# RIVM-bioinformatics/auriclass

Measured on AMD Instinct MI355X. Metric: Gbases/s sketched (k=21, s=1000), higher is better.
Workload: dtype u64; 1 GPU; synthetic FASTQ 10000000 x 150 bp reads per GPU from a 12000000 bp genome, 0.5% substitutions, 3150000000 bytes resident in HBM; k=21, s=1000, min_multiplicity=1, total_bases=1500000000, ranks=1, parallelism=1 GPU

## Files before the change

auriclass_amd/csrc/mhx_sketch.hip:

```cpp
#include "mhx_block.h"
#include "mhx_device.h"
#include "mhx_screen.h"
#include "mhx_tile.h"

#include <type_traits>

namespace mhx {

struct DeviceInserter {
    unsigned long long *keys;
    uint32_t *cnts;
    uint64_t mask;
    unsigned long long *stats;
    __device__ __forceinline__ void operator()(uint64_t h)
    {
        if (h == kEmptyKey) {
            atomicAdd(&stats[kStatMaxKey], 1ull);
            return;
        }
        uint64_t slot = h & mask;
        for (int probe = 0; probe < 8192; ++probe) {
            const unsigned long long prev = atomicCAS(&keys[slot], (unsigned long long)kEmptyKey, (unsigned long long)h);
            if (prev == kEmptyKey || prev == h) {
                atomicAdd(&cnts[slot], 1u);
                return;
            }
            slot = (slot + 1) & mask;
        }
        atomicOr(&stats[kStatFlags], (unsigned long long)kFlagTableFull);
    }
};

struct ScreenProber {
    unsigned long long *keys;
    uint32_t *cnts;
    uint64_t mask;
    unsigned long long *stats;
    __device__ __forceinline__ void operator()(uint64_t h)
    {
        if (h == kEmptyKey) {
            atomicAdd(&stats[kStatMaxKey], 1ull);
            return;
        }
        const uint64_t at = screen_find(reinterpret_cast<const uint64_t *>(keys), mask, h);
        if (at != kScreenAbsent && !screen_count_stands(atomicAdd(&cnts[at], 1u))) {
            atomicSub(&cnts[at], 1u);
            atomicOr(&stats[kStatFlags], (unsigned long long)kFlagCountWrap);
        }
    }
};

template <int K, class Ins> __device__ __noinline__ uint32_t finish_candidate(const TileSmem &sm, uint32_t code, uint64_t T, Ins ins)
{
    return process_deferred<K>(sm, code, T, ins);
}

struct CandidateQueue {
    TileSmem &sm;
    uint32_t first, cap;
    __device__ __forceinline__ void operator()(uint32_t group, int window) const
    {
        const uint32_t slot = atomicAdd(&sm.misc[7], 1u);
        if (slot < cap) sm.list[first + slot] = (uint16_t)((group << 3) | (uint32_t)window);
    }
};

__device__ __forceinline__ uint64_t ld_state(const uint64_t *p)
{
    return __hip_atomic_load(p, __ATOMIC_RELAXED, __HIP_MEMORY_SCOPE_AGENT);
}
__device__ __forceinline__ void st_state(uint64_t *p, uint64_t v)
{
    __hip_atomic_store(p, v, __ATOMIC_RELAXED, __HIP_MEMORY_SCOPE_AGENT);
}

__device__ uint32_t lookback_wave(uint64_t *state, uint32_t tile, uint32_t first_tile, uint32_t agg,
                                  unsigned long long *stats)
{
    const int lane = threadIdx.x & 63;
    constexpr uint64_t A = 1ull << 32, P = 2ull << 32;
    if (tile == first_tile) {
        if (lane == 0) st_state(&state[tile], P | agg);
        return 0;
    }
    if (lane == 0) st_state(&state[tile], A | agg);
    uint32_t excl = 0;
    int64_t pos = (int64_t)tile - 1;
    constexpr int kWin = 4;
    bool done = false;
    for (uint32_t spins = 0; !done;) {
        uint64_t w[kWin];
#pragma unroll
        for (int j = 0; j < kWin; ++j) {
            const int64_t idx = pos - lane - 64 * j;
            w[j] = idx >= (int64_t)first_tile ? ld_state(&state[idx]) : P;
        }
        bool blocked = false;
#pragma unroll
        for (int j = 0; j < kWin; ++j) {
            if (done || blocked) continue;
            const uint32_t f = (uint32_t)(w[j] >> 32);
            const uint64_t notready = __ballot(f == 0);
            const uint64_t isp = __ballot(f == 2);
            uint64_t take = 0;
            if (isp) {
                const int q = __builtin_ctzll(isp);
                const uint64_t below = q ? (~0ull >> (64 - q)) : 0ull;
                if ((notready & below) == 0) {
                    take = below | (1ull << q);
                    done = true;
                }
            } else if (!notready) {
                take = ~0ull;
            }
            if (take) {
                uint32_t v = ((take >> lane) & 1ull) ? (uint32_t)w[j] : 0u;
#pragma unroll
                for (int o = 32; o > 0; o >>= 1) v += __shfl_xor(v, o);
                excl += v;
                if (!done) pos -= 64;
            } else {
                blocked = true;
            }
        }
        if (blocked) {
            if (++spins > (1u << 20)) {
                if (lane == 0) atomicOr(&stats[kStatFlags], (unsigned long long)kFlagSpinTimeout);
                break;
            }
            __builtin_amdgcn_s_sleep(4);
        }
    }
    if (lane == 0) st_state(&state[tile], P | (uint64_t)(excl + agg));
    return excl;
}

#ifdef MHX_PARSE_LOOPS
constexpr bool kParseLoops = true;
#else
constexpr bool kParseLoops = false;
#endif
#ifndef MHX_MIN_WAVES
#define MHX_MIN_WAVES 7
#endif
template <int K, int FMT, bool QUEUE, bool PROBE, bool SPLIT = false> __global__ __launch_bounds__(kBlock, MHX_MIN_WAVES) void sketch_tile_kernel(const HashArgs a)
{
    __shared__ TileSmem sm;
    constexpr bool FASTQ = (FMT != 0), LOOKBACK = (FMT == 1), SELFSYNC = (FMT == 2);
    const int tid = threadIdx.x;
    __builtin_amdgcn_s_setprio(3);

    static_assert(!SPLIT || (!LOOKBACK && !QUEUE && !PROBE), "split launches: inline sketch kernels of formats 0 and 2");
    const uint32_t split_log2 = SPLIT ? (uint32_t)__builtin_ctz(a.split) : 0u;
    const uint32_t slice = SPLIT ? blockIdx.x & (a.split - 1u) : 0u;
    const uint32_t it0 = slice * kBlock + (uint32_t)tid, it_step = (uint32_t)kBlock << split_log2;
    const bool once = slice == 0;
    uint32_t tile;
    if (LOOKBACK) {
        if (tid == 0) sm.misc[2] = a.tile0 + atomicAdd(a.ticket, 1u);
        __syncthreads();
        tile = sm.misc[2];
    } else {
        tile = a.tile0 + (blockIdx.x >> split_log2);
    }
    const uint64_t tile_off = (uint64_t)tile * kTileBytes;
    unsigned long long *stats = reinterpret_cast<unsigned long long *>(a.stats) + (tile % kStatReplicas) * kStatCount;
    if (tid == 0) { sm.misc[3] = 0; sm.misc[4] = 0; sm.misc[5] = 0; sm.misc[7] = 0; }
#ifdef MHX_STAMPS
    uint64_t stamp_prev = clock64();
    int stamp_idx = 0;
#define MHX_STAMP()                                                                                      \
    do {                                                                                                 \
        if (tid == 0) {                                                                                  \
            const uint64_t now_ = clock64();                                                             \
            atomicAdd(&stats[kStatStamp0 + stamp_idx], (unsigned long long)(now_ - stamp_prev));         \
            stamp_prev = now_;                                                                           \
        }                                                                                                \
        ++stamp_idx;                                                                                     \
    } while (0)
#else
#define MHX_STAMP() do { } while (0)
#endif

    phase_stage(sm, tid, a.base, tile_off, a.end);
    __syncthreads();
    MHX_STAMP();

    ThreadState st;
    const bool interior = tile_off >= a.begin && tile_off + kTileBytes + kHaloBytes <= a.end;
    phase_classify(sm, tid, st, tile_off, a.begin, a.end, interior);

    MHX_STAMP();
    uint32_t line_base = 0, excl = 0, tile_total = 0;
    bool fast_parse = false;
    const uint64_t span_left = a.end > tile_off ? a.end - tile_off : 0;
    const uint32_t check_limit = span_left < (uint64_t)(kTileBytes + kHaloBytes) ? (uint32_t)span_left : (uint32_t)(kTileBytes + kHaloBytes);
    if (FASTQ) {
        excl = block_scan_excl<kBlock>(st.nlcount, sm.cnt, tile_total);
        fast_parse = !kParseLoops && parse_events_fit(tile_total);
        if (fast_parse) phase_events(sm, tid, st, excl);
        if (tid == 0) sm.misc[0] = tile == a.first_tile ? 0u : phase_selfsync(sm, check_limit);
        __syncthreads();
        const uint32_t self_phase = sm.misc[0];
        if (SELFSYNC) {
            if (self_phase == 4u) {
                if (tid == 0 && once) { a.phase_rec[tile - a.first_tile] = 0; atomicOr(a.need_lookback, 1u); }
                return;
            }
            if (tid == 0 && once) a.phase_rec[tile - a.first_tile] = phase_record(self_phase, tile_total);
            line_base = self_phase;
        } else {
            if (a.repair && self_phase != 4u) {
                if (tid == 0) {
                    st_state(&a.tile_state[tile], (2ull << 32) | (uint64_t)(self_phase + tile_total));
                    a.phase_rec[tile - a.first_tile] = phase_record(self_phase, tile_total);
                }
                return;
            }
            if (tid < 64) {
                const uint32_t lb = lookback_wave(a.tile_state, tile, a.first_tile, tile_total, stats);
                if (tid == 0) sm.misc[0] = lb;
            }
            __syncthreads();
            line_base = sm.misc[0];
            if (a.repair && tid == 0) a.phase_rec[tile - a.first_tile] = phase_record(line_base, tile_total);
        }
    }
    MHX_STAMP();
    bool bad = false;
    const uint32_t long_records = fast_parse
        ? phase_good_events(sm, tid, st, line_base, excl, tile_total, check_limit, bad, tile_off, a.end, (uint32_t)K)
        : phase_good<FASTQ>(sm, tid, st, line_base, excl, tile_total, check_limit, bad, tile_off, a.end, (uint32_t)K);
    if (FASTQ && bad && once) atomicOr(&stats[kStatFlags], (unsigned long long)kFlagBadFastq);
    if (FASTQ && long_records) atomicAdd(&sm.misc[5], long_records);
    __syncthreads();
    MHX_STAMP();

    uint32_t items = 0;
    const uint32_t kmers = phase_runs<K>(sm, tid, items);
    if (kmers) atomicAdd(&sm.misc[3], kmers);
    uint32_t nitems = 0;
    const uint32_t items_before = block_scan_excl<kBlock>(items, sm.cnt + 8, nitems);
    phase_compact(sm, tid, items_before);
    __syncthreads();
    MHX_STAMP();
    __builtin_amdgcn_s_setprio(0);

    const uint64_t T = *a.thresh;
    const uint32_t limit = admission_limit(T);
    std::conditional_t<PROBE, ScreenProber, DeviceInserter> ins{reinterpret_cast<unsigned long long *>(a.keys), a.cnts, a.slot_mask, stats};
    const uint32_t qcap = (uint32_t)kGroupsPerTile - nitems;
    CandidateQueue queue{sm, nitems, qcap};
    uint32_t ninsert = 0;
    const TailLutPtr lut = hot_tail_table<K>();
    constexpr bool kPairs = pair_words_form<K>(FMT, QUEUE);
    for (uint32_t it = it0; it < nitems; it += it_step) ninsert += process_group<K, QUEUE, kPairs>(sm, sm.list[it], T, limit, ins, queue, lut);
    if (QUEUE) {
        __syncthreads();
        const uint32_t ncand = sm.misc[7];
        if (ncand <= qcap) {
            for (uint32_t c = tid; c < ncand; c += kBlock) ninsert += finish_candidate<K>(sm, sm.list[nitems + c], T, ins);
        } else {
            for (uint32_t it = it0; it < nitems; it += it_step) {
                const uint32_t g = sm.list[it];
                uint32_t vmask = reinterpret_cast<const uint8_t *>(sm.valid)[g];
                while (vmask) {
                    const uint32_t j = (uint32_t)__builtin_ctz(vmask);
                    vmask &= vmask - 1u;
                    ninsert += finish_candidate<K>(sm, (g << 3) | j, T, ins);
                }
            }
        }
    }
    if (ninsert) atomicAdd(&sm.misc[4], ninsert);
    __syncthreads();
    MHX_STAMP();
    if (tid == 0) {
        if (once && sm.misc[3]) atomicAdd(&stats[kStatKmers], (unsigned long long)sm.misc[3]);
        if (sm.misc[4]) atomicAdd(&stats[kStatInserts], (unsigned long long)sm.misc[4]);
        if (once && FASTQ && tile_total) atomicAdd(&stats[kStatLines], (unsigned long long)tile_total);
        if (once && FASTQ && sm.misc[5]) atomicAdd(&stats[kStatRecords], (unsigned long long)sm.misc[5]);
    }
}

template <int K> static hipError_t launch_k(int fmt, const HashArgs &a, hipStream_t st)
{
    if (a.split > 1) {
        if (fmt == 1 || a.queue_candidates || a.probe) return hipErrorInvalidValue;
        if (fmt == 2) hipLaunchKernelGGL((sketch_tile_kernel<K, 2, false, false, true>), dim3(a.ntiles * a.split), dim3(kBlock), 0, st, a);
        else hipLaunchKernelGGL((sketch_tile_kernel<K, 0, false, false, true>), dim3(a.ntiles * a.split), dim3(kBlock), 0, st, a);
        return hipGetLastError();
    }
    const unsigned grid = a.ntiles;
#define MHX_LAUNCH_FORM(FMT_, QUEUE_) do { if (a.probe) hipLaunchKernelGGL((sketch_tile_kernel<K, FMT_, QUEUE_, true>), dim3(grid), dim3(kBlock), 0, st, a); \
                                           else hipLaunchKernelGGL((sketch_tile_kernel<K, FMT_, QUEUE_, false>), dim3(grid), dim3(kBlock), 0, st, a); } while (0)
#define MHX_LAUNCH(FMT_) do { if (a.queue_candidates) MHX_LAUNCH_FORM(FMT_, true); else MHX_LAUNCH_FORM(FMT_, false); } while (0)
    if (fmt == 1) MHX_LAUNCH(1);
    else if (fmt == 2) MHX_LAUNCH(2);
    else MHX_LAUNCH(0);
#undef MHX_LAUNCH
#undef MHX_LAUNCH_FORM
    return hipGetLastError();
}

#ifdef MHX_ONLY_K
#define MHX_K_LIST(X) X(MHX_ONLY_K)
#else
#define MHX_K_LIST(X) X(1) X(2) X(3) X(4) X(5) X(6) X(7) X(8) X(9) X(10) X(11) X(12) X(13) X(14) X(15) X(16) \
    X(17) X(18) X(19) X(20) X(21) X(22) X(23) X(24) X(25) X(26) X(27) X(28) X(29) X(30) X(31) X(32)
#endif

bool hash_k_supported(int k) { return k >= 1 && k <= 32; }

hipError_t launch_hash(int k, int fmt, const HashArgs &a, hipStream_t st)
{
    if (a.ntiles == 0) return hipSuccess;
    if (a.split == 0 || (a.split & (a.split - 1)) || a.split > 8 || (uint64_t)a.ntiles * a.split > 0x7FFFFFFFull) return hipErrorInvalidValue;
    switch (k) {
#define X(KK) case KK: return launch_k<KK>(fmt, a, st);
        MHX_K_LIST(X)
#undef X
    default: return hipErrorInvalidValue;
    }
}

}
```

auriclass_amd/csrc/mhx_tile.h:

```cpp
#pragma once
#include <stdint.h>
#include <type_traits>

#include "mhx_hd.h"
#include "mhx_device_consts.h"
#include "mhx_tail_lut.h"

#define MHX_UNLIKELY(x) __builtin_expect(!!(x), 0)

namespace mhx {

constexpr int kMapWords = (kTileBytes + kHaloBytes) / 32 + 2;
struct TileSmem {
    uint4 bytes[(kTileBytes + kHaloBytes) / 16];
    uint32_t valid[kGroupsPerTile / 4];
    union {
        uint16_t list[kGroupsPerTile];
        uint32_t maps[2 * kMapWords];
    };
    uint32_t cnt[16];
    uint32_t misc[8];
};

MHX_HD uint32_t *tile_nlmap(TileSmem &sm) { return sm.maps; }
// ... 199 lines not shown
{
    const uint32_t lo = (uint32_t)k, hi = (uint32_t)(k >> 32);
    return make64(lo ^ (hi >> 1), hi);
}
MHX_HD uint64_t times5_plus(uint64_t h, uint32_t c)
{
#if defined(__HIP_DEVICE_COMPILE__)
    uint64_t r;
    asm("v_lshl_add_u64 %0, %1, 2, %1" : "=v"(r) : "v"(h));
    return r + c;
#else
    const uint32_t lo = (uint32_t)h, hi = (uint32_t)(h >> 32);
    const uint64_t t = (uint64_t)lo * 5u + c;
    return make64((uint32_t)t, ((hi << 2) + hi) + (uint32_t)(t >> 32));
#endif
}
MHX_HD uint64_t rotated(uint64_t x) { return opaque64(x); }
template <uint64_t C> MHX_HD uint64_t mul64c(uint64_t x, uint32_t &zero)
{
#if defined(__HIP_DEVICE_COMPILE__) && defined(MHX_ASM_MUL64)
    const uint32_t lo = (uint32_t)x, hi = (uint32_t)(x >> 32);
    uint64_t p, carry;
    uint32_t y;
    asm("v_mul_lo_u32 v71, %[lo], %[chi]\n\t"
        "v_mul_lo_u32 %[y], %[hi], %[clo]\n\t"
        "v_add_u32_e32 v71, v71, %[y]\n\t"
        "v_mad_u64_u32 %[p], %[c], %[lo], %[clo], v[70:71]"
        : [p] "=&v"(p), [c] "=&s"(carry), [y] "=&v"(y), "+{v70}"(zero)
        : [lo] "v"(lo), [hi] "v"(hi), [clo] "s"((uint32_t)C), [chi] "s"((uint32_t)(C >> 32))
        : "v71");
    return p;
#else
    (void)zero;
    return opaque64(x * C);
#endif
}
constexpr uint64_t kFmixC2 = 0xc4ceb9fe1a85ec53ull;
MHX_HD uint64_t fmix64_head(uint64_t k, uint32_t &zero)
{
    k = xorshift33(k);
    k = mul64c<0xff51afd7ed558ccdull>(k, zero);
    return xorshift33(k);
}
struct Murmur3Tail {
    uint64_t ka, kb;
    MHX_HD uint64_t finish() const
    {
        uint32_t zero = 0;
        return xorshift33(mul64c<kFmixC2>(ka, zero)) + xorshift33(mul64c<kFmixC2>(kb, zero));
    }
    MHX_HD uint32_t low32() const
    {
        uint32_t zero = 0;
        return (uint32_t)xorshift33(mul64c<kFmixC2>(ka, zero)) + (uint32_t)xorshift33(mul64c<kFmixC2>(kb, zero));
    }
    MHX_HD uint32_t high_bound() const { return (uint32_t)(((ka + kb) * kFmixC2) >> 32) + 1u; }
};
MHX_HD uint32_t admission_limit(uint64_t T)
{
    const uint32_t th = (uint32_t)(T >> 32);
    return th >= 0xFFFFFFFDu ? 0xFFFFFFFFu : th + 2u;
}
template <int K> MHX_HD uint64_t xor_tail_len(uint64_t h, uint64_t k)
{
    h = opaque64(h);
    return make64(xor3((uint32_t)h, (uint32_t)k, (uint32_t)K), (uint32_t)(h >> 32) ^ (uint32_t)(k >> 32));
}
constexpr uint64_t kMurmurSeed = 42;
template <int K> constexpr bool tail_lut_applies() { return K > 16 && (K & 7) >= 1 && (K & 7) <= 5; }
template <int K> constexpr bool hot_tail_lut()
{
#if defined(__HIP_DEVICE_COMPILE__) && !defined(MHX_NO_TAIL_LUT)
    return tail_lut_applies<K>();
#else
    return false;
#endif
}
template <int K> MHX_HD TailLutPtr tail_lut_of() { return tail_lut_table<K & 7, ((K & 15) > 8)>(); }
template <int K, bool LUT> MHX_HD Murmur3Tail murmur3_blocks(const uint32_t (&w)[8], uint64_t k_lut)
{
    static_assert(!LUT || tail_lut_applies<K>(), "no table for this K");
    constexpr uint64_t c1 = kMurmurC1, c2 = kMurmurC2;
    constexpr int NBLK = K / 16, TAIL = K & 15;
    uint64_t h1 = kMurmurSeed, h2 = kMurmurSeed;
    uint32_t zero = 0;
#pragma unroll
    for (int b = 0; b < NBLK; ++b) {
        uint64_t k1 = make64(w[4 * b], w[4 * b + 1]);
        uint64_t k2 = make64(w[4 * b + 2], w[4 * b + 3]);
        k1 = rotl64<31>(mul64c<c1>(k1, zero)); k1 = mul64c<c2>(k1, zero); h1 ^= k1;
        h1 = rotated(rotl64<27>(h1));
        static_assert(0x52dce729ull + 5ull * kMurmurSeed <= 0xFFFFFFFFull, "folded constant of block 0 must fit times5_plus' 32-bit addend");
        if (b == 0) h1 = times5_plus(h1, (uint32_t)(0x52dce729ull + 5ull * kMurmurSeed));
        else { h1 += h2; h1 = times5_plus(h1, 0x52dce729u); }
        k2 = rotl64<33>(mul64c<c2>(k2, zero)); k2 = mul64c<c1>(k2, zero); h2 ^= k2;
        h2 = rotated(rotl64<31>(h2)); h2 += h1; h2 = times5_plus(h2, 0x38495ab5u);
    }
    if (TAIL > 8) {
        uint64_t k2 = make64(w[(4 * NBLK + 2) & 7], w[(4 * NBLK + 3) & 7]);
        if constexpr (LUT) k2 = k_lut;
        else { k2 = rotl64<33>(mul64c<c2>(k2, zero)); k2 = mul64c<c1>(k2, zero); }
        h2 = xor_tail_len<K>(h2, k2);
    } else {
        h2 ^= (uint64_t)K;
    }
    if (TAIL > 0) {
        uint64_t k1 = make64(w[(4 * NBLK) & 7], w[(4 * NBLK + 1) & 7]);
        if constexpr (LUT && TAIL <= 8) k1 = k_lut;
        else { k1 = rotl64<31>(mul64c<c1>(k1, zero)); k1 = mul64c<c2>(k1, zero); }
        h1 = xor_tail_len<K>(h1, k1);
    } else {
        h1 ^= (uint64_t)K;
    }
    h1 += h2; h2 += h1;
    uint64_t ka = fmix64_head(h1, zero), kb = fmix64_head(h2, zero);
    if (K > 16) { ka = opaque64(ka); kb = opaque64(kb); }
    return Murmur3Tail{ka, kb};
}
template <int K, bool LUT = false> MHX_HD Murmur3Tail murmur3_core(const uint32_t (&w)[8], TailLutPtr lut = nullptr)
{
    uint64_t k_lut = 0;
    if constexpr (LUT) k_lut = lut[tail_lut_index<K & 7>(w[(K / 8) * 2], w[((K / 8) * 2 + 1) & 7])];
    return murmur3_blocks<K, LUT>(w, k_lut);
}
template <int K> MHX_HD uint64_t murmur3_h1(const uint32_t (&w)[8]) { return murmur3_core<K>(w).finish(); }


MHX_HD void phase_stage(TileSmem &sm, int tid, const uint8_t *base, uint64_t tile_off, uint64_t end)
{
    const uint64_t lim = (end + 15) & ~(uint64_t)15;
    constexpr int kChunks = kTileBytes / 16;
#ifndef MHX_STAGE_SERIAL
    if (tile_off + (uint64_t)(kTileBytes + kHaloBytes) <= lim) {
        const uint4 *src = reinterpret_cast<const uint4 *>(base + tile_off) + tid;
        uint4 v[kChunks / kBlock], h = {0, 0, 0, 0};
#pragma unroll
        for (int j = 0; j < kChunks / kBlock; ++j) v[j] = src[j * kBlock];
        if (tid < kHaloBytes / 16) h = src[kChunks];
#pragma unroll
        for (int j = 0; j < kChunks / kBlock; ++j) sm.bytes[j * kBlock + tid] = v[j];
        if (tid < kHaloBytes / 16) sm.bytes[kChunks + tid] = h;
        return;
    }
#endif
#pragma unroll
    for (int j = 0; j < kChunks / kBlock; ++j) {
        const int c = j * kBlock + tid;
        const uint64_t off = tile_off + (uint64_t)c * 16;
        uint4 v = {0, 0, 0, 0};
        if (off < lim) v = *reinterpret_cast<const uint4 *>(base + off);
        sm.bytes[c] = v;
    }
    if (tid < kHaloBytes / 16) {
        const int c = kChunks + tid;
        const uint64_t off = tile_off + (uint64_t)c * 16;
        uint4 v = {0, 0, 0, 0};
        if (off < lim) v = *reinterpret_cast<const uint4 *>(base + off);
        sm.bytes[c] = v;
    }
}

MHX_HD void phase_classify(TileSmem &sm, int tid, ThreadState &st, uint64_t tile_off, uint64_t begin, uint64_t end, bool interior)
{
    const uint32_t *p = reinterpret_cast<const uint32_t *>(sm.bytes) + tid * (kBytesPerThread / 4);
    uint32_t total = 0;
#pragma unroll
    for (int w = 0; w < kWordsPerThread; ++w) {
        st.in[w] = interior ? 0xFFFFFFFFu : inrange_mask(tile_off + (uint64_t)tid * kBytesPerThread + 32u * w, begin, end);
        st.nl[w] = newline_mask(p + 8 * w) & st.in[w];
        total += (uint32_t)__builtin_popcount(st.nl[w]);
        tile_nlmap(sm)[tid * kWordsPerThread + w] = st.nl[w];
    }
    st.nlcount = total;
    if (tid == 0) {
        const uint32_t *h = reinterpret_cast<const uint32_t *>(sm.bytes) + kTileBytes / 4;
#pragma unroll
        for (int w = 0; w < 2; ++w) {
            st.hin[w] = interior ? 0xFFFFFFFFu : inrange_mask(tile_off + kTileBytes + 32u * w, begin, end);
            st.hnl[w] = newline_mask(h + 8 * w) & st.hin[w];
            tile_nlmap(sm)[kTileBytes / 32 + w] = st.hnl[w];
        }
    }
}


MHX_HD uint32_t phase_selfsync(TileSmem &sm, uint32_t check_limit)
{
    const uint32_t *nlmap = tile_nlmap(sm);
    const uint8_t *b = reinterpret_cast<const uint8_t *>(sm.bytes);
    uint32_t pos[6];
    int n = 0;
    for (int w = 0; w < kTileBytes / 32 + 2 && n < 6; ++w) {
        uint32_t m = nlmap[w];
        while (m && n < 6) {
            pos[n++] = 32u * (uint32_t)w + (uint32_t)__builtin_ctz(m);
            m &= m - 1u;
        }
    }
    for (int i = 0; i + 2 < n && i < 4; ++i) {
        const uint32_t p0 = pos[i] + 1u, p1 = pos[i + 1] + 1u, p2 = pos[i + 2] + 1u;
        if (p2 >= check_limit) break;
        if (b[p0] == '@' && b[p1] != '@' && b[p1] != '+' && b[p2] == '+') return (4u - ((uint32_t)(i + 1) & 3u)) & 3u;
    }
    return 4u;
}

constexpr uint8_t kPhaseKnown = 0x10;
MHX_HD uint8_t phase_record(uint32_t start_phase, uint32_t tile_lines)
{
    return (uint8_t)(kPhaseKnown | (start_phase & 3u) | (((start_phase + tile_lines) & 3u) << 2));
}
MHX_HD bool phase_chain_broken(uint8_t prev, uint8_t cur)
{
    return (prev & kPhaseKnown) && (cur & kPhaseKnown) && ((prev >> 2) & 3u) != (cur & 3u);
}

template <bool FASTQ>
MHX_HD uint32_t phase_good(TileSmem &sm, int tid, const ThreadState &st, uint32_t line_base, uint32_t excl,
                           uint32_t tile_total, uint32_t check_limit, bool &bad_format, uint64_t tile_off, uint64_t end, uint32_t k)
{
    const uint8_t *tb = reinterpret_cast<const uint8_t *>(sm.bytes);
    LineLenCheck lc{tile_nlmap(sm), tile_off, end, k, 0u};
    uint32_t line = line_base + excl;
#pragma unroll
    for (int w = 0; w < kWordsPerThread; ++w) {
        uint32_t g;
        if (FASTQ) {
            g = st.in[w] & seqline_mask(st.nl[w], line, tb, (uint32_t)tid * kBytesPerThread + 32u * w, check_limit, bad_format, &lc);
            line += (uint32_t)__builtin_popcount(st.nl[w]);
        } else {
            g = st.in[w] & ~st.nl[w];
        }
        tile_good(sm)[tid * kWordsPerThread + w] = g;
    }
    if (tid == 0) {
        uint32_t hl = line_base + tile_total;
#pragma unroll
        for (int w = 0; w < 2; ++w) {
            uint32_t g;
            if (FASTQ) {
                bool ignore = false;
                g = st.hin[w] & seqline_mask(st.hnl[w], hl, nullptr, 0, 0, ignore);
                hl += (uint32_t)__builtin_popcount(st.hnl[w]);
            } else {
                g = st.hin[w] & ~st.hnl[w];
            }
            tile_good(sm)[kTileBytes / 32 + w] = g;
        }
        tile_good(sm)[kTileBytes / 32 + 2] = 0;
        tile_good(sm)[kTileBytes / 32 + 3] = 0;
    }
    return lc.count;
}

constexpr uint32_t kEventCap = kGroupsPerTile / 2;
static_assert(kEventCap * 2 == sizeof(TileSmem::valid) && kEventCap % kBlock == 0, "event list = sm.valid");
static_assert(kTileBytes + kHaloBytes <= 65536, "event positions are 16-bit");
MHX_HD bool parse_events_fit(uint32_t tile_total) { return tile_total <= kEventCap; }

MHX_HD uint32_t prefix_parity_excl(uint32_t x)
{
    x ^= x << 1; x ^= x << 2; x ^= x << 4; x ^= x << 8; x ^= x << 16;
    return x << 1;
}
MHX_HD uint32_t seqline_mask_bits(uint32_t nl, uint32_t line)
{
    const uint32_t b0 = prefix_parity_excl(nl) ^ (0u - (line & 1u));
    const uint32_t b1 = prefix_parity_excl(nl & b0) ^ (0u - ((line >> 1) & 1u));
    return b0 & ~b1 & ~nl;
}

MHX_HD void phase_events(TileSmem &sm, int tid, const ThreadState &st, uint32_t excl)
{
    uint16_t *ev = reinterpret_cast<uint16_t *>(sm.valid);
    uint32_t at = excl;
#pragma unroll
    for (int w = 0; w < kWordsPerThread; ++w) {
        const uint32_t off = (uint32_t)tid * kBytesPerThread + 32u * w;
        uint32_t nl = st.nl[w];
        if (nl) {
            ev[at] = (uint16_t)(off + (uint32_t)__builtin_ctz(nl));
            nl &= nl - 1u;
            if (nl) {
                ev[at + 1u] = (uint16_t)(off + (uint32_t)__builtin_ctz(nl));
                nl &= nl - 1u;
                for (uint32_t j = 2; MHX_UNLIKELY(nl != 0); ++j, nl &= nl - 1u) ev[at + j] = (uint16_t)(off + (uint32_t)__builtin_ctz(nl));
            }
        }
        at += (uint32_t)__builtin_popcount(st.nl[w]);
    }
}

MHX_HD bool seqline_is_long(const uint32_t *nlmap, const uint8_t *tile_bytes, uint32_t pos, uint64_t tile_off, uint64_t end, uint32_t k)
{
    const uint32_t wq = pos >> 5, sh = pos & 31u;
    const uint32_t window = funnel_bits(nlmap[wq + 1], nlmap[wq], sh);
    const uint32_t first_k = k >= 32 ? 0xFFFFFFFFu : ((1u << k) - 1u);
    if ((window & first_k) != 0 || tile_off + pos + k > end) return false;
    const uint32_t after = pos + k;
    const bool ends_here = tile_off + after >= end || ((nlmap[after >> 5] >> (after & 31u)) & 1u);
    return !(tile_bytes[after - 1u] == '\r' && ends_here);
}

MHX_HD uint32_t phase_good_events(TileSmem &sm, int tid, const ThreadState &st, uint32_t line_base, uint32_t excl,
                                  uint32_t tile_total, uint32_t check_limit, bool &bad_format, uint64_t tile_off, uint64_t end, uint32_t k)
{
    uint32_t line = line_base + excl;
#pragma unroll
    for (int w = 0; w < kWordsPerThread; ++w) {
        tile_good(sm)[tid * kWordsPerThread + w] = st.in[w] & seqline_mask_bits(st.nl[w], line);
        line += (uint32_t)__builtin_popcount(st.nl[w]);
    }
    if (tid == 0) {
        uint32_t hl = line_base + tile_total;
#pragma unroll
        for (int w = 0; w < 2; ++w) {
            tile_good(sm)[kTileBytes / 32 + w] = st.hin[w] & seqline_mask_bits(st.hnl[w], hl);
            hl += (uint32_t)__builtin_popcount(st.hnl[w]);
        }
        tile_good(sm)[kTileBytes / 32 + 2] = 0;
        tile_good(sm)[kTileBytes / 32 + 3] = 0;
    }
    const uint8_t *tb = reinterpret_cast<const uint8_t *>(sm.bytes);
    const uint16_t *ev = reinterpret_cast<const uint16_t *>(sm.valid);
    uint32_t count = 0;
#pragma unroll
    for (uint32_t r = 0; r < kEventCap / kBlock; ++r) {
        if (r == 1 && tile_total <= (uint32_t)kBlock) break;
        const uint32_t e = r * kBlock + (uint32_t)tid;
        if (e < tile_total) {
            const uint32_t pos = (uint32_t)ev[e] + 1u;
            const uint32_t idx = (line_base + e + 1u) & 3u;
            if (idx == 1u) {
                if (seqline_is_long(tile_nlmap(sm), tb, pos, tile_off, end, k)) ++count;
            } else if (idx != 3u && pos < check_limit) {
                if (tb[pos] != (idx == 0u ? '@' : '+')) bad_format = true;
            }
        }
    }
    return count;
}

template <int K> MHX_HD uint32_t phase_runs(TileSmem &sm, int tid, uint32_t &items_out)
{
    constexpr int NWD = kWordsPerThread;
    uint32_t w[NWD + 1], v[NWD];
#pragma unroll
    for (int i = 0; i < NWD + 1; ++i) w[i] = tile_good(sm)[tid * NWD + i];
    run_starts<K, NWD>(w, v);
    uint32_t items = 0, kmers = 0;
#pragma unroll
    for (int i = 0; i < NWD; ++i) {
        sm.valid[tid * NWD + i] = v[i];
        kmers += (uint32_t)__builtin_popcount(v[i]);
        items += 4u - (uint32_t)__builtin_popcount(zero_byte_flags(v[i]));
    }
    items_out = items;
    return kmers;
}

MHX_HD void phase_compact(TileSmem &sm, int tid, uint32_t excl)
{
    uint32_t pos = excl;
#pragma unroll
    for (int i = 0; i < kWordsPerThread; ++i) {
        const uint32_t v = sm.valid[tid * kWordsPerThread + i];
#pragma unroll
        for (int b = 0; b < 4; ++b)
            if ((v >> (8 * b)) & 0xFFu) sm.list[pos++] = (uint16_t)((tid * kWordsPerThread + i) * 4 + b);
    }
    if (tid == kBlock - 1) sm.misc[1] = pos;
}

MHX_HD uint32_t complement4(uint32_t u) { return perm_lut(kLutComp, base_index(u)); }

template <int OFF, int N> MHX_HD uint64_t load64(const uint32_t (&a)[N])
{
    constexpr int q = OFF / 4, sh = OFF % 4;
    static_assert(q + (sh ? 2 : 1) < N, "load64 out of range");
    const uint32_t lo = sh ? funnel(a[q + 1], a[q], sh) : a[q];
    const uint32_t hi = sh ? funnel(a[q + 2], a[q + 1], sh) : a[q + 1];
    return ((uint64_t)hi << 32) | lo;
}

template <int NW> MHX_HD bool rc_is_smaller_full(const uint32_t (&wf)[8], const uint32_t (&wr)[8])
{
    bool rc_less = false, decided = false;
#pragma unroll
    for (int i = 0; i < NW; ++i) {
        const uint32_t a = __builtin_bswap32(wf[i]), b = __builtin_bswap32(wr[i]);
        rc_less = decided ? rc_less : (b < a);
        decided = decided || (a != b);
    }
    return rc_less;
}

template <int K, int OFF, int N> MHX_HD void extract_words(const uint32_t (&src)[N], uint32_t (&w)[8])
{
    constexpr int NW = (K + 3) / 4;
#pragma unroll
    for (int i = 0; i < 8; ++i) w[i] = i < NW ? funnel(src[OFF / 4 + i + 1], src[OFF / 4 + i], OFF % 4) : 0u;
    if (K % 4) w[NW - 1] &= (1u << (8 * (K % 4))) - 1u;
}

template <int K, int J, int ND>
MHX_HD bool canonical_strand(const uint32_t (&U)[ND + 1], const uint32_t (&R)[ND + 1])
{
    static_assert(K >= 8, "shorter windows compare their extracted words");
    constexpr int NW = (K + 3) / 4;
    constexpr int OF = J;
    constexpr int OR = ND * 4 - K - J;
    static_assert(J >= 0 && J + K <= 4 * ND, "the window lies inside the chunk");
    static_assert(J + K - 8 >= 0 && J + K <= 4 * (ND + 1), "A: 8 bytes inside U[0..ND]");
    static_assert(4 * ND - 8 - J >= 0 && 4 * ND - J <= 4 * (ND + 1), "B: 8 bytes inside R[0..ND]");
    if constexpr (K == 8 && J % 4 == 0) {
        constexpr int QA = J / 4, QB = ND - 2 - J / 4;
        return R[QB + 1] < U[QA + 1] || (R[QB + 1] == U[QA + 1] && R[QB] < U[QA]);
    }
    const uint64_t top_a = load64<J + K - 8>(U);
    const uint64_t top_b = load64<ND * 4 - 8 - J>(R);
    bool rc = top_b < top_a;
    if (MHX_UNLIKELY(K > 8 && top_a == top_b)) {
        uint32_t Uc[ND + 1], Rc[ND + 1];
#pragma unroll
        for (int i = 0; i < ND + 1; ++i) { Uc[i] = opaque(U[i]); Rc[i] = opaque(R[i]); }
        constexpr uint32_t last_mask = (K % 4) ? (1u << (8 * (K % 4))) - 1u : 0xFFFFFFFFu;
        bool rc_less = false, decided = false;
#pragma unroll
        for (int i = 0; i < NW; ++i) {
            uint32_t f = funnel(Uc[OF / 4 + i + 1], Uc[OF / 4 + i], OF % 4);
            uint32_t r = funnel(Rc[OR / 4 + i + 1], Rc[OR / 4 + i], OR % 4);
            if (i == NW - 1) { f &= last_mask; r &= last_mask; }
            const uint32_t fb = opaque(__builtin_bswap32(f)), rb = opaque(__builtin_bswap32(r));
            rc_less = decided ? rc_less : (rb < fb);
            decided = decided || (fb != rb);
        }
        rc = rc_less;
    }
    return rc;
}
template <int K, int J, int ND>
MHX_HD bool canonical_strand(const uint32_t (&U)[ND + 1], const uint32_t (&R)[ND + 1], const uint32_t (&)[ND + 1], const uint32_t (&)[ND + 1])
{
    return canonical_strand<K, J, ND>(U, R);
}

template <int K, int J, int ND, bool BODY_ONLY = false>
MHX_HD bool canonical_words(const uint32_t (&U)[ND + 1], const uint32_t (&R)[ND + 1], uint32_t (&w)[8])
{
    static_assert(!BODY_ONLY || K > 16, "the body-only form belongs to the tail table (64-bit hashes)");
    constexpr int NW = (K + 3) / 4;
    constexpr int OF = J;
    constexpr int OR = ND * 4 - K - J;
    if constexpr (K >= 8) {
        const bool rc = canonical_strand<K, J, ND>(U, R);
        if constexpr (BODY_ONLY) {
            constexpr int NBW = 2 * (K / 8);
            static_assert(NBW < NW, "a partial word follows the body");
            uint32_t S[NBW + 1];
#pragma unroll
            for (int i = 0; i < NBW + 1; ++i) S[i] = rc ? R[OR / 4 + i] : U[OF / 4 + i];
            const uint32_t sh = rc ? 8u * (OR % 4) : 8u * (OF % 4);
#pragma unroll
            for (int i = 0; i < 8; ++i) w[i] = i < NBW ? funnel_bits(S[i + 1], S[i], sh) : 0u;
        } else {
            constexpr int TB = K - 4 * (NW - 1);
            constexpr bool need_f = OF % 4 + TB > 4, need_r = OR % 4 + TB > 4;
            uint32_t S[NW];
#pragma unroll
            for (int i = 0; i < NW; ++i) S[i] = rc ? R[OR / 4 + i] : U[OF / 4 + i];
            const uint32_t sh = rc ? 8u * (OR % 4) : 8u * (OF % 4);
#pragma unroll
            for (int i = 0; i < 8; ++i)
                w[i] = i < NW - 1 ? funnel_bits(S[i + 1], S[i], sh) : 0u;
            if constexpr (!need_f && !need_r) {
                if constexpr (TB == 4) w[NW - 1] = S[NW - 1];
                else w[NW - 1] = bit_field<8 * TB>(S[NW - 1], sh);
            } else {
                const uint32_t last = need_f && need_r ? (rc ? R[OR / 4 + NW] : U[OF / 4 + NW]) : need_f ? U[OF / 4 + NW] : R[OR / 4 + NW];
                w[NW - 1] = funnel_bits(last, S[NW - 1], sh);
                if constexpr (TB < 4) w[NW - 1] &= (1u << (8 * TB)) - 1u;
            }
        }
        return rc;
    } else {
        uint32_t wf[8], wr[8];
        extract_words<K, OF>(U, wf);
        extract_words<K, OR>(R, wr);
        const bool rc = rc_is_smaller_full<NW>(wf, wr);
#pragma unroll
        for (int i = 0; i < 8; ++i) w[i] = rc ? wr[i] : wf[i];
        return rc;
    }
}
template <int K, int J, int ND, bool BODY_ONLY = false>
MHX_HD bool canonical_words(const uint32_t (&U)[ND + 1], const uint32_t (&R)[ND + 1], const uint32_t (&)[ND + 1], const uint32_t (&)[ND + 1],
                            uint32_t (&w)[8])
{
    return canonical_words<K, J, ND, BODY_ONLY>(U, R, w);
}

template <int K> struct GroupGeom {
    static constexpr int NB = kGroup + K - 1;
    static constexpr int ND = (NB + 3) / 4;
};

constexpr uint32_t kLutComp8Lo = 0x00470054u, kLutComp8Hi = 0x00430041u;
MHX_HD uint32_t complement_lut_lo()
{
    uint32_t lo = kLutComp8Lo;
#if defined(__HIP_DEVICE_COMPILE__)
    asm("" : "+v"(lo));
#endif
    return lo;
}
MHX_HD uint32_t complement4_raw(uint32_t v, uint32_t lut_lo)
{
#if defined(__HIP_DEVICE_COMPILE__)
    return __builtin_amdgcn_perm(kLutComp8Hi, lut_lo, v & 0x06060606u);
#else
    const uint64_t lut = ((uint64_t)kLutComp8Hi << 32) | lut_lo;
    uint32_t o = 0;
    for (int i = 0; i < 4; ++i) o |= (uint32_t)((lut >> (8 * ((v >> (8 * i)) & 6u))) & 0xFFu) << (8 * i);
    return o;
#endif
}

template <int ND> MHX_HD void strand_views(const uint32_t (&src)[ND], uint32_t (&U)[ND + 1], uint32_t (&R)[ND + 1])
{
    const uint32_t lut_lo = complement_lut_lo();
#pragma unroll
    for (int d = 0; d < ND; ++d) {
        U[d] = src[d] & 0xDFDFDFDFu;
        R[d] = __builtin_bswap32(complement4_raw(src[ND - 1 - d], lut_lo));
    }
    U[ND] = R[ND] = 0;
}
template <int ND>
MHX_HD void strand_views(const uint32_t (&src)[ND], uint32_t (&U)[ND + 1], uint32_t (&R)[ND + 1], uint32_t (&Wr)[ND + 1], uint32_t (&Cc)[ND + 1])
{
    strand_views<ND>(src, U, R);
#pragma unroll
    for (int d = 0; d < ND; ++d) {
        Wr[d] = __builtin_bswap32(U[ND - 1 - d]);
        Cc[d] = __builtin_bswap32(R[ND - 1 - d]);
    }
    Wr[ND] = Cc[ND] = 0;
}

template <int K> struct TailDigits {
    static constexpr int T = K & 7, Q = K / 8, ND = GroupGeom<K>::ND;
    static constexpr int NDW = (T + 7 + 3) / 4;
    static constexpr int FD = 2 * Q;
    static constexpr int RD = ND - NDW;
    static_assert(T >= 1 && T <= 5 && NDW <= 3, "partial words of 1..5 bases: 8..12 bytes per strand");
    static_assert(FD + NDW <= ND + 1 && RD >= 0, "the packed dwords lie inside U[0..ND] and R[0..ND)");
    static_assert(4 * ND - K - 7 + 8 * Q >= 4 * RD, "reverse window 7 starts inside the packed dwords");
    static_assert(7 + 8 * Q + T <= 4 * (FD + NDW), "forward window 7 ends inside the packed dwords");
    template <int J> static constexpr uint32_t shift_f() { return 2u * J; }
    template <int J> static constexpr uint32_t shift_r() { return 2u * (uint32_t)(4 * ND - K - J + 8 * Q - 4 * RD); }
    uint64_t both;
    MHX_HD TailDigits(const uint32_t (&U)[ND + 1], const uint32_t (&R)[ND + 1])
        : both(opaque64(make64(tail_lut_pack<NDW>(U[FD], U[FD + 1], U[FD + NDW - 1]), tail_lut_pack<NDW>(R[RD], R[RD + 1], R[RD + NDW - 1])) << 3)) {}
    template <int J> MHX_HD uint32_t byte_offset(bool rc) const
    {
        static_assert(shift_f<J>() + 2 * T <= 8 * NDW && shift_r<J>() + 2 * T <= 8 * NDW, "the field lies inside the packed word");
        static_assert(8 * NDW + 3 <= 32 && 2 * T + 3 <= 32 - (int)shift_f<7>(), "what the other word shifts in stays above the field");
        uint32_t low = (uint32_t)(both >> (rc ? 32u + shift_r<J>() : shift_f<J>()));
#if defined(__HIP_DEVICE_COMPILE__)
        asm("" : "+v"(low));
#endif
        return low & (((1u << (2 * T)) - 1u) << 3);
    }
};
template <int K> constexpr bool tail_digits_apply() { return K == 21; }
struct NoTailDigits {
    template <class A, class B> MHX_HD NoTailDigits(const A &, const B &) {}
};
template <int K, int J, int ND, bool LUT, class Digits>
MHX_HD Murmur3Tail window_partial_hash(const uint32_t (&U)[ND + 1], const uint32_t (&R)[ND + 1], const Digits &digits, TailLutPtr lut)
{
    uint32_t w[8];
    if constexpr (LUT && std::is_same<Digits, TailDigits<K>>::value) {
        const bool rc = canonical_words<K, J, ND, true>(U, R, w);
        return murmur3_blocks<K, true>(w, tail_lut_at(lut, digits.template byte_offset<J>(rc)));
    } else {
        canonical_words<K, J, ND>(U, R, w);
        return murmur3_core<K, LUT>(w, lut);
    }
}
template <int K, int J, int ND, bool LUT, class Digits>
MHX_HD Murmur3Tail window_partial_hash(const uint32_t (&U)[ND + 1], const uint32_t (&R)[ND + 1], const uint32_t (&)[ND + 1],
                                       const uint32_t (&)[ND + 1], const Digits &digits, TailLutPtr lut)
{
    return window_partial_hash<K, J, ND, LUT>(U, R, digits, lut);
}

template <int K, int J, int ND, bool BODY_ONLY> struct PairWords {
    static constexpr int NW = (K + 3) / 4;
    static constexpr int NWD = BODY_ONLY ? 2 * (K / 8) : NW;
    static constexpr int OF = J, OR = 4 * ND - K - J;
    static constexpr int SF = OF % 4, SR = OR % 4;
    static constexpr int FD = OF / 4, RD = OR / 4 - 1;
    static_assert(J >= 0 && J < 4 && K > 16, "pairs (J, J + 4) of the 64-bit hashes");
    static_assert(NWD > 0 && NWD <= 8 && 4 * NWD <= K + 3, "the dwords made lie inside the window");
    static_assert((OF + 4) % 4 == SF && (OF + 4) / 4 == FD + 1, "forward window J + 4 starts one dword behind window J");
    static_assert(OR - 4 >= 0 && (OR - 4) % 4 == SR && (OR - 4) / 4 == RD, "reverse window J + 4 starts at byte OR - 4 >= 0, one dword in front");
    static_assert(FD + NWD + (SF ? 1 : 0) <= ND && RD + NWD + (SR ? 1 : 0) <= ND, "the source dwords lie inside U[0..ND] and R[0..ND]");
    uint32_t F[NWD + 1], G[NWD + 1];
    MHX_HD PairWords(const uint32_t (&U)[ND + 1], const uint32_t (&R)[ND + 1])
    {
#pragma unroll
        for (int i = 0; i < NWD + 1; ++i) {
            F[i] = SF ? funnel(U[FD + i + 1], U[FD + i], SF) : U[FD + i];
            G[i] = SR ? funnel(R[RD + i + 1], R[RD + i], SR) : R[RD + i];
        }
    }
    template <bool SECOND> MHX_HD void words(bool rc, uint32_t (&w)[8]) const
    {
#pragma unroll
        for (int i = 0; i < 8; ++i) w[i] = i < NWD ? (rc ? G[i + (SECOND ? 0 : 1)] : F[i + (SECOND ? 1 : 0)]) : 0u;
        if constexpr (!BODY_ONLY && K % 4 != 0) w[NW - 1] &= (1u << (8 * (K % 4))) - 1u;
    }
};
template <int K> constexpr bool pair_words_apply()
{
    return K == 17 || K == 18 || K == 19 || K == 21 || K == 23 || K == 25 || K == 26 || K == 27 || K == 29;
}
template <int K> constexpr bool pair_words_form(int fmt, bool queue)
{
    return pair_words_apply<K>() && (K > 24 ? queue : fmt != 1 || queue);
}
template <int K, int J, int ND, bool SECOND, bool LUT, bool BODY_ONLY, class Digits>
MHX_HD Murmur3Tail window_pair_hash(const PairWords<K, J, ND, BODY_ONLY> &pair, const uint32_t (&U)[ND + 1], const uint32_t (&R)[ND + 1],
                                    const Digits &digits, TailLutPtr lut)
{
    constexpr int JW = J + (SECOND ? 4 : 0);
    uint32_t w[8];
    const bool rc = canonical_strand<K, JW, ND>(U, R);
    pair.template words<SECOND>(rc, w);
    if constexpr (BODY_ONLY) {
        static_assert(LUT && std::is_same<Digits, TailDigits<K>>::value, "the body-only form takes the table index from packed digits");
        return murmur3_blocks<K, true>(w, tail_lut_at(lut, digits.template byte_offset<JW>(rc)));
// ... 124 lines not shown
```

Before: 438.2 Gbases/s.

## Build k-mer items directly from sequence line spans on interior tiles

For FASTQ interior tiles with few sequence lines, each lane of one wave takes one sequence line, computes its valid k-mer start span from newline events, and writes the item list and validity bytes directly. This skips building the per-thread good-bit map, run_starts, the block-wide scan and compaction. If any line's span exceeds a group limit, the code falls back to the map path, paying an extra barrier. The cost is serial per-line item writing by at most 64 lanes, while the rest of the block sits idle.

```diff
diff --git a/auriclass_amd/csrc/mhx_sketch.hip b/auriclass_amd/csrc/mhx_sketch.hip
--- a/auriclass_amd/csrc/mhx_sketch.hip
+++ b/auriclass_amd/csrc/mhx_sketch.hip
@@ -165,6 +165,7 @@
     }
     const uint64_t tile_off = (uint64_t)tile * kTileBytes;
     unsigned long long *stats = reinterpret_cast<unsigned long long *>(a.stats) + (tile % kStatReplicas) * kStatCount;
+    constexpr bool kLineItems = !kParseLoops && line_items_form<K>(FMT, QUEUE);
     if (tid == 0) { sm.misc[3] = 0; sm.misc[4] = 0; sm.misc[5] = 0; sm.misc[7] = 0; }
 #ifdef MHX_STAMPS
     uint64_t stamp_prev = clock64();
@@ -228,21 +229,48 @@
     }
     MHX_STAMP();
     bool bad = false;
-    const uint32_t long_records = fast_parse
-        ? phase_good_events(sm, tid, st, line_base, excl, tile_total, check_limit, bad, tile_off, a.end, (uint32_t)K)
-        : phase_good<FASTQ>(sm, tid, st, line_base, excl, tile_total, check_limit, bad, tile_off, a.end, (uint32_t)K);
+    bool by_lines = kLineItems && line_items_try(fast_parse, interior, line_base, tile_total);
+    uint32_t long_records, items_at = 0;
+    LineSpan span{0u, 0u, 0u, 0u};
+    if (kLineItems && by_lines) {
+        long_records = phase_event_checks(sm, tid, line_base, tile_total, check_limit, bad, tile_off, a.end, (uint32_t)K);
+        if (tid < (int)kLineItemLines) {
+            span = phase_line_span<K>(sm, (uint32_t)tid, line_base, tile_total);
+            const bool too_long = __ballot(line_span_too_long(span)) != 0ull;
+            if (tid == 0) { sm.misc[1] = 0u; sm.misc[6] = too_long ? 1u : 0u; }
+            items_at = atomicAdd(&sm.misc[1], span.ngroups);
+        }
+    } else {
+        long_records = fast_parse
+            ? phase_good_events(sm, tid, st, line_base, excl, tile_total, check_limit, bad, tile_off, a.end, (uint32_t)K)
+            : phase_good<FASTQ>(sm, tid, st, line_base, excl, tile_total, check_limit, bad, tile_off, a.end, (uint32_t)K);
+    }
     if (FASTQ && bad && once) atomicOr(&stats[kStatFlags], (unsigned long long)kFlagBadFastq);
     if (FASTQ && long_records) atomicAdd(&sm.misc[5], long_records);
     __syncthreads();
     MHX_STAMP();
-
-    uint32_t items = 0;
-    const uint32_t kmers = phase_runs<K>(sm, tid, items);
-    if (kmers) atomicAdd(&sm.misc[3], kmers);
+    if (kLineItems && by_lines && MHX_UNLIKELY(sm.misc[6] != 0u)) {
+        by_lines = false;
+        phase_good_events_map(sm, tid, st, line_base, excl, tile_total);
+        __syncthreads();
+    }
+
     uint32_t nitems = 0;
-    const uint32_t items_before = block_scan_excl<kBlock>(items, sm.cnt + 8, nitems);
-    phase_compact(sm, tid, items_before);
-    __syncthreads();
+    if (kLineItems && by_lines) {
+        if (tid < (int)kLineItemLines) {
+            if (span.kmers) atomicAdd(&sm.misc[3], span.kmers);
+            phase_line_items(sm, span, items_at);
+        }
+        __syncthreads();
+        nitems = sm.misc[1];
+    } else {
+        uint32_t items = 0;
+        const uint32_t kmers = phase_runs<K>(sm, tid, items);
+        if (kmers) atomicAdd(&sm.misc[3], kmers);
+        const uint32_t items_before = block_scan_excl<kBlock>(items, sm.cnt + 8, nitems);
+        phase_compact(sm, tid, items_before);
+        __syncthreads();
+    }
     MHX_STAMP();
     __builtin_amdgcn_s_setprio(0);
 
diff --git a/auriclass_amd/csrc/mhx_tile.h b/auriclass_amd/csrc/mhx_tile.h
--- a/auriclass_amd/csrc/mhx_tile.h
+++ b/auriclass_amd/csrc/mhx_tile.h
@@ -525,8 +525,7 @@
     return !(tile_bytes[after - 1u] == '\r' && ends_here);
 }
 
-MHX_HD uint32_t phase_good_events(TileSmem &sm, int tid, const ThreadState &st, uint32_t line_base, uint32_t excl,
-                                  uint32_t tile_total, uint32_t check_limit, bool &bad_format, uint64_t tile_off, uint64_t end, uint32_t k)
+MHX_HD void phase_good_events_map(TileSmem &sm, int tid, const ThreadState &st, uint32_t line_base, uint32_t excl, uint32_t tile_total)
 {
     uint32_t line = line_base + excl;
 #pragma unroll
@@ -544,6 +543,10 @@
         tile_good(sm)[kTileBytes / 32 + 2] = 0;
         tile_good(sm)[kTileBytes / 32 + 3] = 0;
     }
+}
+MHX_HD uint32_t phase_event_checks(TileSmem &sm, int tid, uint32_t line_base, uint32_t tile_total, uint32_t check_limit,
+                                   bool &bad_format, uint64_t tile_off, uint64_t end, uint32_t k)
+{
     const uint8_t *tb = reinterpret_cast<const uint8_t *>(sm.bytes);
     const uint16_t *ev = reinterpret_cast<const uint16_t *>(sm.valid);
     uint32_t count = 0;
@@ -562,6 +565,76 @@
         }
     }
     return count;
+}
+MHX_HD uint32_t phase_good_events(TileSmem &sm, int tid, const ThreadState &st, uint32_t line_base, uint32_t excl,
+                                  uint32_t tile_total, uint32_t check_limit, bool &bad_format, uint64_t tile_off, uint64_t end, uint32_t k)
+{
+    phase_good_events_map(sm, tid, st, line_base, excl, tile_total);
+    return phase_event_checks(sm, tid, line_base, tile_total, check_limit, bad_format, tile_off, end, k);
+}
+
+constexpr uint32_t kLineItemLines = 64;
+constexpr uint32_t kLineItemGroups = 40;
+constexpr uint32_t kLineItemMinNewlines = 48;
+static_assert(kLineItemLines <= 64, "the sequence lines of a tile take the lanes of one wave");
+template <int K> constexpr bool line_items_apply()
+{
+#ifdef MHX_PARSE_MAPS
+    return false;
+#else
+    return K >= 8;
+#endif
+}
+template <int K> constexpr bool line_items_form(int fmt, bool queue) { return line_items_apply<K>() && fmt == 2 && !(K == 29 && queue); }
+MHX_HD uint32_t seqline_first(uint32_t line_base) { return (1u - line_base) & 3u; }
+MHX_HD uint32_t seqline_count(uint32_t line_base, uint32_t tile_total)
+{
+    const uint32_t i0 = seqline_first(line_base);
+    return i0 <= tile_total ? (tile_total - i0) / 4u + 1u : 0u;
+}
+MHX_HD bool line_items_try(bool fast_parse, bool interior, uint32_t line_base, uint32_t tile_total)
+{
+    return fast_parse && interior && tile_total >= kLineItemMinNewlines && seqline_count(line_base, tile_total) <= kLineItemLines;
+}
+struct LineSpan { uint32_t a, pmax, ngroups, kmers; };
+template <int K> MHX_HD LineSpan phase_line_span(const TileSmem &sm, uint32_t j, uint32_t line_base, uint32_t tile_total)
+{
+    const uint16_t *ev = reinterpret_cast<const uint16_t *>(sm.valid);
+    const uint32_t i = seqline_first(line_base) + 4u * j;
+    LineSpan s{0u, 0u, 0u, 0u};
+    if (i > tile_total) return s;
+    const uint32_t a = i ? (uint32_t)ev[i - 1u] + 1u : 0u;
+    uint32_t b;
+    if (i < tile_total) {
+        b = ev[i];
+    } else {
+        const uint32_t h0 = sm.maps[kTileBytes / 32], h1 = sm.maps[kTileBytes / 32 + 1];
+        b = h0 ? (uint32_t)kTileBytes + (uint32_t)__builtin_ctz(h0) : h1 ? (uint32_t)kTileBytes + 32u + (uint32_t)__builtin_ctz(h1) : (uint32_t)(kTileBytes + kHaloBytes);
+    }
+    int32_t pmax = (int32_t)b - K;
+    if (pmax > kTileBytes - 1) pmax = kTileBytes - 1;
+    if (pmax < (int32_t)a) return s;
+    s.a = a;
+    s.pmax = (uint32_t)pmax;
+    s.ngroups = ((uint32_t)pmax >> 3) - (a >> 3) + 1u;
+    s.kmers = (uint32_t)pmax - a + 1u;
+    return s;
+}
+MHX_HD bool line_span_too_long(const LineSpan &s) { return s.ngroups > kLineItemGroups; }
+MHX_HD void phase_line_items(TileSmem &sm, const LineSpan &s, uint32_t at)
+{
+    if (!s.ngroups) return;
+    uint8_t *vb = reinterpret_cast<uint8_t *>(sm.valid);
+    const uint32_t g0 = s.a >> 3, g1 = s.pmax >> 3;
+    const uint32_t first = (0xFFu << (s.a & 7u)) & 0xFFu, last = 0xFFu >> (7u - (s.pmax & 7u));
+    sm.list[at] = (uint16_t)g0;
+    vb[g0] = (uint8_t)(g0 == g1 ? first & last : first);
+    if (g0 == g1) return;
+    for (uint32_t g = g0 + 1u; g <= g1; ++g) {
+        sm.list[++at] = (uint16_t)g;
+        vb[g] = 0xFFu;
+    }
+    vb[g1] = (uint8_t)last;
 }
 
 template <int K> MHX_HD uint32_t phase_runs(TileSmem &sm, int tid, uint32_t &items_out)
```

New measurement: 460.8 Gbases/s (median of 6 runs). +5.2%, better.
